# intel/QATzip

Measured on AMD Instinct MI355X. Metric: compress + decompress GB/s (input bytes), QZ_DEFLATE_GZIP_EXT L1, 64 KB chunks, higher is better.
Workload: dtype u8

## Files before the change

### qatzip_amd/csrc/qzk_common.h

```cpp
#ifndef QZK_COMMON_H
#define QZK_COMMON_H
#include <stdint.h>

#ifdef QZ_SIM
#include "hipsim.h"
#define QZ_DEV static inline
#define QZ_KERNEL static void
#define QZ_KERNEL_MAX(n) static void
#define QZ_KERNEL_OCC(n, w) static void
#define QZ_LDS static
#define QZ_CONST static const
#else
#include <hip/hip_runtime.h>
#define QZ_DEV static __device__ __forceinline__
#define QZ_KERNEL static __global__ void
#define QZ_KERNEL_MAX(n) static __global__ void __launch_bounds__(n)
#define QZ_KERNEL_OCC(n, w) static __global__ void __launch_bounds__(n, w)
#define QZ_LDS __shared__
#define QZ_CONST static __device__ const

QZ_DEV uint64_t qz_ballot(bool p) { return __ballot(p); }
QZ_DEV uint32_t qz_shfl(uint32_t v, int src) { return (uint32_t)__shfl((int)v, src, 64); }
QZ_DEV uint32_t qz_readlane(uint32_t v, int src) { return (uint32_t)__builtin_amdgcn_readlane((int)v, src); }
QZ_DEV uint32_t qz_readfirstlane(uint32_t v) { return (uint32_t)__builtin_amdgcn_readfirstlane((int)v); }
QZ_DEV uint32_t qz_writelane(uint32_t old, uint32_t val, int sel) { return (int)(threadIdx.x & 63) == sel ? val : old; }
QZ_DEV void qz_wave_sync()
{
    __builtin_amdgcn_fence(__ATOMIC_RELEASE, "workgroup");
    __builtin_amdgcn_wave_barrier();
    __builtin_amdgcn_fence(__ATOMIC_ACQUIRE, "workgroup");
}
QZ_DEV void qz_lds_sync()
{
    __builtin_amdgcn_fence(__ATOMIC_ACQ_REL, "wavefront");
    __builtin_amdgcn_wave_barrier();
}
QZ_DEV void qz_block_sync() { __syncthreads(); }
QZ_DEV int qz_lane() { return (int)(threadIdx.x & 63); }
QZ_DEV uint8_t qz_ld8_l2(const uint8_t *p) { return __hip_atomic_load(p, __ATOMIC_RELAXED, __HIP_MEMORY_SCOPE_AGENT); }
#endif
#ifdef QZ_SIM
static inline void qz_lds_sync() { qz_wave_sync(); }
static inline uint32_t qz_writelane(uint32_t old, uint32_t val, int sel) { return qz_lane() == sel ? val : old; }
static inline uint8_t qz_ld8_l2(const uint8_t *p) { return *p; }
#endif

#ifndef QZ_SIM
QZ_DEV uint32_t qz_wave_incl_scan(uint32_t v)
{
    v += (uint32_t)__builtin_amdgcn_update_dpp(0, (int)v, 0x111, 0xf, 0xf, false);
    v += (uint32_t)__builtin_amdgcn_update_dpp(0, (int)v, 0x112, 0xf, 0xf, false);
    v += (uint32_t)__builtin_amdgcn_update_dpp(0, (int)v, 0x114, 0xf, 0xf, false);
    v += (uint32_t)__builtin_amdgcn_update_dpp(0, (int)v, 0x118, 0xf, 0xf, false);
    v += (uint32_t)__builtin_amdgcn_update_dpp(0, (int)v, 0x142, 0xa, 0xf, false);
    v += (uint32_t)__builtin_amdgcn_update_dpp(0, (int)v, 0x143, 0xc, 0xf, false);
    return v;
}
#else
static inline uint32_t qz_wave_incl_scan(uint32_t v)
{
    const int lane = qz_lane();
    for (int d = 1; d < 64; d <<= 1) {
        uint32_t o = qz_shfl(v, lane - d);
        if (lane >= d) v += o;
    }
    return v;
}
#endif

QZ_DEV int qz_popc64(uint64_t v) { return __builtin_popcountll(v); }
QZ_DEV int qz_ctz64(uint64_t v) { return __builtin_ctzll(v); }
QZ_DEV int qz_ctz32(uint32_t v) { return __builtin_ctz(v); }
QZ_DEV int qz_msb64(uint64_t v) { return 63 - __builtin_clzll(v); }
QZ_DEV uint64_t qz_below(int l) { return l >= 64 ? ~0ull : ((1ull << l) - 1); }

typedef struct __attribute__((packed, aligned(1))) { uint32_t v; } qz_u32u;
typedef struct __attribute__((packed, aligned(1))) { uint16_t v; } qz_u16u;
QZ_DEV uint32_t qz_ld32(const uint8_t *p) { return ((const qz_u32u *)p)->v; }
QZ_DEV uint32_t qz_ld16(const uint8_t *p) { return ((const qz_u16u *)p)->v; }

QZ_DEV uint32_t qz_uniform(uint32_t v) { return qz_readfirstlane(v); }

#endif
```

### qatzip_amd/csrc/qzk_deflate_lz77.h

```cpp
#ifndef QZK_DEFLATE_LZ77_H
#define QZK_DEFLATE_LZ77_H
#include "qzk_common.h"
#include "qzk_crcmath.h"

#define QZK_WSIZE 32768
#define QZK_MAXDIST 32506
#define QZK_MINLOOK 262
#define QZK_LITBUF 32767
#define QZK_MAXBLK 20
#define QZK_CAP 16
#define QZK_WLIM 61
#define QZK_NICE 8
#define QZK_MAXINS 4
#define QZK_HSIZE 65536
#ifndef QZK_CNBLOG
#define QZK_CNBLOG (-1)
#endif
#if QZK_CNBLOG >= 0
#define QZK_CNB (1 << QZK_CNBLOG)
#else
#define QZK_CNB 0
#endif
#ifndef QZK_PF
#define QZK_PF (QZK_CNB ? 1 : 0)
#endif
#ifndef QZK_PF_MINL
#define QZK_PF_MINL 30
#endif
#ifndef QZK_NSLOT
#define QZK_NSLOT 256
#endif
#ifndef QZK_RING
#define QZK_RING 4096
#endif
#ifndef QZK_K1_OCC
#define QZK_K1_OCC 5
#endif
#define QZK_RINGW (QZK_RING / 4)
#ifndef QZK_NSLOT2
#define QZK_NSLOT2 128
#endif
#ifndef QZK_NSLOT3
#if QZK_CNB
#define QZK_NSLOT3 0
#else
#define QZK_NSLOT3 128
#endif
#endif
#define QZK_K1_PARSEW (2 * QZK_NSLOT + QZK_RINGW + 4 + QZK_NSLOT2 + QZK_NSLOT3 + 3 * QZK_CNB)
#ifndef QZK_K1_WAVES
#define QZK_K1_WAVES 4
#endif

#ifndef QZK_K1_TABGRP
#define QZK_K1_TABGRP 5
#endif
#define QZK_K1_TABW (QZK_K1_WAVES * QZK_K1_TABGRP)
#define QZK_K1_TABROWS(wgs) ((((wgs) + 8u * QZK_K1_TABGRP - 1) / (8u * QZK_K1_TABGRP)) * 8u)

typedef struct __attribute__((aligned(16))) { uint32_t w0, w1, w2, ep; } qzk_bkt;
typedef uint32_t qzk_u32x4 __attribute__((vector_size(16)));

QZ_DEV qzk_u32x4 qzk_ld_bkt(const qzk_bkt *p)
{
#ifdef QZ_SIM
    return *(const qzk_u32x4 *)p;
#else
    qzk_u32x4 v;
    asm volatile("global_load_dwordx4 %0, %1, off sc1\n\ts_waitcnt vmcnt(0)" : "=v"(v) : "v"(p) : "memory");
    return v;
#endif
}

QZ_DEV void qzk_ld_bkt_ahead(qzk_u32x4 *v, const qzk_bkt *p)
{
#ifdef QZ_SIM
    *v = *(const qzk_u32x4 *)p;
#else
    asm volatile("global_load_dwordx4 %0, %1, off sc1" : "+v"(*v) : "v"(p) : "memory");
#endif
}
QZ_DEV void qzk_wait_ahead(qzk_u32x4 *v)
{
#ifdef QZ_SIM
    (void)v;
#else
    asm volatile("s_waitcnt vmcnt(0)" : "+v"(*v) : : "memory");
#endif
}

#ifdef QZ_SIM
static unsigned long qzk_sim_count[2];
#define QZK_SIMC(k) do { if (qz_lane() == 0) qzk_sim_count[k]++; } while (0)
#else
#define QZK_SIMC(k) do { } while (0)
#endif
#if defined(QZK_PROF) && !defined(QZ_SIM)
#define QZK_T(k) do { uint64_t t_ = __builtin_readcyclecounter(); prof[k] += t_ - tprev; tprev = t_; } while (0)
#define QZK_C(k, v) do { prof[k] += (uint64_t)(v); } while (0)
#else
#define QZK_T(k) do { } while (0)
#define QZK_C(k, v) do { } while (0)
#endif

typedef struct {
    uint32_t nsym;
    uint32_t nfull;
    uint32_t bstart[QZK_MAXBLK];
    uint32_t can_store;
    uint32_t n;
#ifdef QZK_PROF
    uint64_t prof[24];
#endif
} qzk_lzmeta;

#define QZK_CDESC_FINAL 0x80000000u
QZ_DEV uint32_t qzk_chunk_len(const uint32_t *cdesc, uint32_t chunk, uint64_t src_len, uint32_t chunk_sz)
{
    if (cdesc) return cdesc[chunk] & ~QZK_CDESC_FINAL;
    const uint64_t coff = (uint64_t)chunk * chunk_sz;
    return (uint32_t)((src_len - coff) < chunk_sz ? (src_len - coff) : chunk_sz);
}

QZ_DEV uint32_t qzk_ld32g(const uint8_t *src, uint64_t off, uint64_t src_len)
{
    if (off + 4 <= src_len) return qz_ld32(src + off);
    uint32_t v = 0;
    for (int k = 0; k < 4; k++) if (off + k < src_len) v |= (uint32_t)src[off + k] << (8 * k);
    return v;
}

QZ_DEV uint32_t qzk_ld32g_fast(const uint8_t *src, uint64_t off, uint64_t src_len)
{
    return off + 4 <= src_len ? qz_ld32(src + off) : qzk_ld32g(src, off, src_len);
}

QZ_DEV uint32_t qzk_alignbyte(uint32_t hi, uint32_t lo, uint32_t s)
{
#ifdef QZ_SIM
    return (uint32_t)((((uint64_t)hi << 32) | lo) >> (8 * s));
#else
    return __builtin_amdgcn_alignbyte(hi, lo, s);
#endif
}

QZ_DEV int qzk_wave_matchlen(const uint8_t *src, uint64_t src_len, uint64_t a, uint64_t b, int maxlen, int lane)
{
    for (int off = 0; off < maxlen; off += 256) {
        int o = off + 4 * lane;
        bool act = o < maxlen;
        uint32_t x = 0;
        if (act) x = qzk_ld32g(src, a + o, src_len) ^ qzk_ld32g(src, b + o, src_len);
        uint64_t mm = qz_ballot(act && x != 0);
        if (mm) {
            int f = qz_ctz64(mm);
            uint32_t xf = qz_readlane(x, f);
            int len = off + 4 * f + (qz_ctz32(xf) >> 3);
            return len < maxlen ? len : maxlen;
        }
    }
    return maxlen;
}

QZ_DEV void qzk_lz77_chunk(const uint8_t *src, uint64_t src_len, uint32_t chunk_sz, uint32_t chunk,
                           uint8_t *sym_lc, uint16_t *sym_dist, qzk_lzmeta *meta, qzk_bkt *tab, uint32_t epoch,
                           const uint32_t *cdesc, uint32_t *lds, const qzk_k1crc_lds *crcT, uint32_t *crc_slot)
{
    uint32_t *const slot = lds, *const scnt = lds + QZK_NSLOT, *const ring = lds + 2 * QZK_NSLOT, *const slot2 = ring + QZK_RINGW + 4;
    uint32_t *const slot3 = slot2 + QZK_NSLOT2; (void)slot3;
#if QZK_CNB
    uint32_t *const ctag = slot3 + QZK_NSLOT3, *const cpos = ctag + QZK_CNB;
#pragma nounroll
    for (uint32_t i = (uint32_t)qz_lane(); i < QZK_CNB; i += 64) ctag[i] = 0;
#endif
    uint32_t rhi = 0;
    uint32_t crc_acc = 0;
    uint32_t rnext = qzk_ld32g_fast(src, (uint64_t)chunk * chunk_sz + 4 * (uint32_t)qz_lane(), src_len);
#define QZK_RING16(dst, ca) do { const uint32_t r_ = (ca) & (QZK_RING - 1), i_ = r_ >> 2, s_ = r_ & 3; \
        const uint32_t d0_ = ring[i_], d1_ = ring[i_ + 1], d2_ = ring[i_ + 2], d3_ = ring[i_ + 3], d4_ = ring[i_ + 4]; \
        (dst)[0] = qzk_alignbyte(d1_, d0_, s_); (dst)[1] = qzk_alignbyte(d2_, d1_, s_); \
        (dst)[2] = qzk_alignbyte(d3_, d2_, s_); (dst)[3] = qzk_alignbyte(d4_, d3_, s_); } while (0)
#define QZK_RING4(ca) ({ const uint32_t r_ = (ca) & (QZK_RING - 1), i_ = r_ >> 2; \
        qzk_alignbyte(ring[i_ + 1], ring[i_], r_ & 3); })
#define QZK_AHEAD (64 + 258 + 6)

    const int lane = qz_lane();
    const uint64_t coff = (uint64_t)chunk * chunk_sz;
    const uint32_t n = qzk_chunk_len(cdesc, chunk, src_len, chunk_sz);
    uint8_t *olc = sym_lc;
    uint16_t *odist = sym_dist;
    qzk_lzmeta *mt = meta + chunk;
    auto wave_matchlen = [&](uint32_t ca, uint32_t cb, int maxlen) -> int {
        const bool near = (int64_t)cb >= (int64_t)rhi - QZK_RING;
        for (int off = 0; off < maxlen; off += 256) {
            const int o = off + 4 * lane;
            const bool act = o < maxlen;
            uint32_t x = 0;
            if (act) x = QZK_RING4(ca + (uint32_t)o) ^ (near ? QZK_RING4(cb + (uint32_t)o) : qzk_ld32g(src, coff + cb + (uint32_t)o, src_len));
            const uint64_t mm = qz_ballot(act && x != 0);
            if (mm) {
                const int f = qz_ctz64(mm);
                const uint32_t xf = qz_readlane(x, f);
                const int len = off + 4 * f + (qz_ctz32(xf) >> 3);
                return len < maxlen ? len : maxlen;
            }
        }
        return maxlen;
    };

    qz_lds_sync();

    uint32_t base = 0;
    uint32_t fill = n < 65536u ? n : 65536u;
    uint32_t avail_in = n - fill;
    uint32_t pos = 0;
    uint32_t nsym = 0, nfull = 0, cur_bstart = 0, can_store = 0;
    mt->bstart[0] = 0;
#if QZK_PF
    qzk_u32x4 pf = {0, 0, 0, 0};
    uint64_t pf_okm = 0;
    uint32_t pf_base = 0, pf_mark = 0, wcount = 0;
    bool pf_lost = false;
    uint64_t dPm = 0, dSTm = 0;
    uint32_t dnsym = 0, dv_sym = 0, dv_h = 0, dv_e0 = 0, dv_e1 = 0, dv_e2 = 0;
#define QZK_DEFERRED_STORES() do { \
        if ((dPm >> lane) & 1) { const uint32_t i_ = dnsym + (uint32_t)qz_popc64(dPm & qz_below(lane)); \
                                 olc[i_] = (uint8_t)dv_sym; odist[i_] = (uint16_t)(dv_sym >> 8); } \
        if ((dSTm >> lane) & 1) { const qzk_u32x4 e_ = {dv_e0, dv_e1, dv_e2, epoch}; *(qzk_u32x4 *)&tab[(size_t)dv_h * QZK_K1_TABW] = e_; } \
        dPm = 0; dSTm = 0; } while (0)
    bool pf_live = false;
#endif
#if defined(QZK_PROF) && !defined(QZ_SIM)
    uint64_t prof[24] = {0}; uint64_t tprev = __builtin_readcyclecounter();
#endif

    for (;;) {
        uint32_t look = fill - pos;
        if (look < QZK_MINLOOK) {
            if (pos - base >= (uint32_t)(QZK_WSIZE + QZK_MAXDIST)) {
                base += QZK_WSIZE;
#if QZK_CNB
                qz_lds_sync();
#pragma nounroll
                for (uint32_t i = (uint32_t)lane; i < 2 * QZK_CNB; i += 64) {
                    const uint32_t v = cpos[i];
                    const int a = (int)(v & 0xffffu) - QZK_WSIZE, b = (int)(v >> 16) - QZK_WSIZE;
                    cpos[i] = (uint32_t)(a > 0 ? a : 0) | (uint32_t)(b > 0 ? b : 0) << 16;
                }
                qz_lds_sync();
#endif
            }
            if (avail_in) {
                uint32_t more = 65536u - (fill - base);
                uint32_t rd = avail_in < more ? avail_in : more;
                fill += rd; avail_in -= rd;
            }
            look = fill - pos;
            if (look == 0) break;
        }

        QZK_T(0); QZK_C(8, 1);
#if QZK_PF
        qzk_wait_ahead(&pf);
        QZK_T(17);
        QZK_DEFERRED_STORES();
        QZK_T(18);
#endif
        const uint32_t B = pos - base;
        const uint32_t p = B + (uint32_t)lane;
        const uint32_t pa = pos + (uint32_t)lane;
        const int avail = pa < fill ? (int)(fill - pa) : 0;
        const bool canh = avail >= 3;
        const bool guard = coff + pos + 64 + 2 * QZK_CAP > src_len;
        uint32_t w0 = 0, w1 = 0, w2 = 0, w3 = 0;
        {
            if (rhi < pos + QZK_AHEAD) {
                do {
                    const uint32_t a = rhi + 4 * (uint32_t)lane;
                    const uint32_t ri = (a >> 2) & (QZK_RINGW - 1);
                    ring[ri] = rnext;
                    if (ri < 4) ring[ri + QZK_RINGW] = rnext;
                    if (crcT && a + 4 <= n) crc_acc = qzk_k1crc_step(crcT, crc_acc, rnext);
                    rhi += 256;
                    rnext = qzk_ld32g_fast(src, coff + a + 256, src_len);
                } while (rhi < pos + QZK_AHEAD);
                qz_lds_sync();
            }
            uint32_t w[4];
            QZK_RING16(w, pa);
            w0 = w[0]; w1 = w[1]; w2 = w[2]; w3 = w[3];
        }
        const uint32_t h = (((w0 & 0xf) << 12) ^ (((w0 >> 8) & 0xff) << 6) ^ ((w0 >> 16) & 0xff)) & 0xffff;
        const uint32_t bucket = h;
        const uint32_t key = h & (QZK_NSLOT - 1);

        int nvalid = look < 64 ? (int)look : 64;
        int lim = nvalid < QZK_WLIM ? nvalid : QZK_WLIM;
        {
            int lstop;
            int first_short = (int)look - (QZK_MINLOOK - 1);
            if (first_short < 0) first_short = 0;
            if (avail_in) lstop = first_short;
            else {
                int sl = (int)(QZK_WSIZE + QZK_MAXDIST) - (int)B;
                lstop = first_short > sl ? first_short : sl;
            }
            if (lstop < 1) lstop = 1;
            if (lim > lstop) lim = lstop;
        }
        QZK_T(1);
        qz_lds_sync();
        qzk_u32x4 ev = {0, 0, 0, 0};
#if QZK_CNB
        const uint32_t cset = ((h * 40503u) >> (16 - QZK_CNBLOG)) & (QZK_CNB - 1);
        const uint32_t ct = ctag[cset], cp0 = cpos[cset], cp1 = cpos[QZK_CNB + cset];
        const bool chit = canh && ct == (h | 0x10000u);
        QZK_C(8, (uint64_t)qz_popc64(qz_ballot(chit)) << 32);
#if QZK_PF
        bool evhave = false;
        int limdata = 64;
        {
            const uint32_t sh = pos - pf_base;
            if (pf_live && !pf_lost && sh < 64u - (QZK_PF_MINL + 3)) {
                const int sl = lane + (int)sh;
                const uint32_t a0 = qz_shfl(pf[0], sl), a1 = qz_shfl(pf[1], sl), a2 = qz_shfl(pf[2], sl), a3 = qz_shfl(pf[3], sl);
                if (canh && !chit && sl < 64 && ((pf_okm >> (sl & 63)) & 1) && slot[key] != (pf_mark | h) && scnt[(h >> 8) & (QZK_NSLOT - 1)] != (pf_mark | h)) {
                    ev[0] = a0; ev[1] = a1; ev[2] = a2; ev[3] = a3; evhave = true;
                }
            }
            const bool lack = canh && !chit && !evhave;
            const uint64_t LACK = qz_ballot(lack);
            if (LACK) {
                const int fl = qz_ctz64(LACK);
                if (fl < QZK_PF_MINL + 3) { if (lack) { ev = qzk_ld_bkt(&tab[(size_t)bucket * QZK_K1_TABW]); evhave = true; } QZK_C(15, 1ull << 32); QZK_SIMC(0); }
                else limdata = fl - 3;
            }
        }
#else
        const bool evhave = canh && !chit;
        if (canh && !chit) ev = qzk_ld_bkt(&tab[(size_t)bucket * QZK_K1_TABW]);
#endif
#if QZK_PF
        if (lim > limdata) lim = limdata;
        QZK_SIMC(1);
#endif
        QZK_T(16);
        const bool ev_ok = ev[3] == epoch;
        uint32_t q0 = ev_ok ? ev[0] & 0xffffffu : 0, q1 = ev_ok ? (ev[0] >> 24) | ((ev[1] & 0xffffu) << 8) : 0,
                 q2 = ev_ok ? (ev[1] >> 16) | ((ev[2] & 0xffu) << 16) : 0, q3 = ev_ok ? ev[2] >> 8 : 0;
        if (chit) {
            q0 = (cp0 & 0xffffu) ? base + (cp0 & 0xffffu) : 0; q1 = (cp0 >> 16) ? base + (cp0 >> 16) : 0;
            q2 = (cp1 & 0xffffu) ? base + (cp1 & 0xffffu) : 0; q3 = (cp1 >> 16) ? base + (cp1 >> 16) : 0;
        }
#else
        if (canh) ev = qzk_ld_bkt(&tab[(size_t)bucket * QZK_K1_TABW]);
        const bool ev_ok = ev[3] == epoch;
        const uint32_t q0 = ev_ok ? ev[0] & 0xffffffu : 0, q1 = ev_ok ? (ev[0] >> 24) | ((ev[1] & 0xffffu) << 8) : 0,
                       q2 = ev_ok ? (ev[1] >> 16) | ((ev[2] & 0xffu) << 16) : 0, q3 = ev_ok ? ev[2] >> 8 : 0;
#endif
        const uint32_t lo = base + (p > QZK_MAXDIST ? p - QZK_MAXDIST : 0);
        const int maxlen = avail < 258 ? avail : 258;
        const int nice = avail < QZK_NICE ? avail : QZK_NICE;
        int best_len = 2; uint32_t best_c = 0;
        int l0 = 0, l1 = 0, l2 = 0, l3 = 0;
        bool suspect;
        int nc; uint32_t c0, c1, c2, c3;
        {
            uint32_t x[4][4];
            const bool ok0 = canh && q0 > base && pa - q0 <= QZK_MAXDIST;
            const bool ok1 = ok0 && q1 > lo;
            const bool ok2 = ok1 && q2 > lo;
            const bool ok3 = ok2 && q3 > lo;
            c0 = ok0 ? q0 : pa; c1 = ok1 ? q1 : pa; c2 = ok2 ? q2 : pa; c3 = ok3 ? q3 : pa;
            QZK_RING16(x[0], c0); QZK_RING16(x[1], c1); QZK_RING16(x[2], c2); QZK_RING16(x[3], c3);
#define QZK_LDF(k, ck) do { const uint32_t ca_ = (ck); if ((int64_t)ca_ < (int64_t)rhi - QZK_RING) { const uint64_t g_ = coff + ca_; \
        if (!guard) { x[k][0] = qz_ld32(src + g_); x[k][1] = qz_ld32(src + g_ + 4); x[k][2] = qz_ld32(src + g_ + 8); x[k][3] = qz_ld32(src + g_ + 12); } \
        else { x[k][0] = qzk_ld32g(src, g_, src_len); x[k][1] = qzk_ld32g(src, g_ + 4, src_len); x[k][2] = qzk_ld32g(src, g_ + 8, src_len); x[k][3] = qzk_ld32g(src, g_ + 12, src_len); } } } while (0)
#ifndef QZK_EXP_NOFAR
            QZK_LDF(0, c0); QZK_LDF(1, c1); QZK_LDF(2, c2); QZK_LDF(3, c3);
#endif
#undef QZK_LDF
            nc = (int)ok0 + (int)ok1 + (int)ok2 + (int)ok3;
            QZK_T(2);
            const uint32_t key2 = (h >> (16 - 8)) & (QZK_NSLOT2 - 1);
#if QZK_NSLOT3
            const uint32_t key3 = ((h * 40503u) >> 12) & (QZK_NSLOT3 - 1);
            if (canh) slot3[key3] = 0xffffffffu;
#endif
            if (canh) { slot[key] = 0xffffffffu; scnt[key] = 0; slot2[key2] = 0xffffffffu; }
            qz_lds_sync();
            if (canh) { atomicMin(&slot[key], ((uint32_t)lane << 16) | h); atomicAdd(&scnt[key], 1u); atomicMin(&slot2[key2], (uint32_t)lane); }
#if QZK_NSLOT3
            if (canh) atomicMin(&slot3[key3], (uint32_t)lane);
#endif
            qz_lds_sync();
            {
                const uint32_t sv = canh ? slot[key] : 0, sc = canh ? scnt[key] : 0, s2 = canh ? slot2[key2] : 0;
                suspect = canh && (sv >> 16) != (uint32_t)lane && !(sc == 2 && (sv & 0xffff) != h) && s2 != (uint32_t)lane;
#if QZK_NSLOT3
                if (suspect && slot3[key3] == (uint32_t)lane) suspect = false;
#endif
            }
            bool done = false;
            for (int k = 0; k < 4; k++) {
                const uint32_t ck = k == 0 ? c0 : k == 1 ? c1 : k == 2 ? c2 : c3;
                int len = 0;
                if (k < nc) {
                    uint32_t d;
                    len = QZK_CAP;
                    d = w3 ^ x[k][3]; if (d) len = 12 + (qz_ctz32(d) >> 3);
                    d = w2 ^ x[k][2]; if (d) len = 8 + (qz_ctz32(d) >> 3);
                    d = w1 ^ x[k][1]; if (d) len = 4 + (qz_ctz32(d) >> 3);
                    d = w0 ^ x[k][0]; if (d) len = (qz_ctz32(d) >> 3);
                    if (len > maxlen) len = maxlen;
                    if (!done) {
                        if (len > best_len) { best_len = len; best_c = ck; }
                        if (len >= nice) done = true;
                    }
                }
                if (k == 0) l0 = len; else if (k == 1) l1 = len; else if (k == 2) l2 = len; else l3 = len;
            }
        }
        uint32_t mlen = best_len >= 3 ? (uint32_t)best_len : 0;
        uint32_t mdist = mlen ? pa - best_c : 0;
        const bool capped = (best_len == QZK_CAP) && (maxlen > QZK_CAP);
        const bool exact0 = nc > 0 && pa - c0 == QZK_MAXDIST;

        QZK_T(3);
        const uint64_t CANH = qz_ballot(canh);
        const uint64_t CAPM = qz_ballot(capped);
        const uint64_t CX = qz_ballot(suspect) | CAPM;
        const uint64_t NOLIT = qz_ballot(mlen != 0) | CX;

        QZK_T(4);
#if QZK_PF
        {
            pf_base = pos + (uint32_t)lim; pf_live = true;
            pf_mark = 0x80000000u | wcount << 16; wcount = (wcount + 1) & 0x7fffu;
            const uint32_t ppa = pf_base + (uint32_t)lane;
            const bool pcanh = ppa + 3 <= fill;
            const uint32_t pw = QZK_RING4(ppa);
            const uint32_t ph = (((pw & 0xf) << 12) ^ (((pw >> 8) & 0xff) << 6) ^ ((pw >> 16) & 0xff)) & 0xffff;
            const uint32_t ps = ((ph * 40503u) >> (16 - QZK_CNBLOG)) & (QZK_CNB - 1);
            const uint32_t pct = ctag[ps], pc0 = cpos[ps], pc1 = cpos[QZK_CNB + ps];
            const uint32_t g0 = (pc0 & 0xffffu) ? base + (pc0 & 0xffffu) : 0, g1 = (pc0 >> 16) ? base + (pc0 >> 16) : 0,
                           g2 = (pc1 & 0xffffu) ? base + (pc1 & 0xffffu) : 0, g3 = (pc1 >> 16) ? base + (pc1 >> 16) : 0;
            pf[0] = g0 | (g1 << 24); pf[1] = (g1 >> 8) | (g2 << 16); pf[2] = (g2 >> 16) | (g3 << 8); pf[3] = epoch;
            if (pcanh && pct != (ph | 0x10000u)) qzk_ld_bkt_ahead(&pf, &tab[(size_t)ph * QZK_K1_TABW]);
            pf_okm = qz_ballot(pcanh);
        }
#endif
        uint64_t Pm = 0;
        uint64_t SHm = qz_ballot(mlen >= 3 && mlen <= QZK_MAXINS && avail - (int)mlen >= 3), S4m = qz_ballot(mlen == 4);
        int l = 0;
        while (l < lim) {
            uint64_t cxr = CX >> l;
            int nextc = cxr ? l + qz_ctz64(cxr) : 64;
            int stop = nextc < lim ? nextc : lim;
            while (l < stop) {
                const uint64_t nl = (NOLIT | (1ull << 63)) >> l;
                int e = l + qz_ctz64(nl);
                if (e > stop) e = stop;
                const uint32_t ml = qz_readlane(mlen, e);
                const int isM = e < stop ? 1 : 0;
                Pm |= ((1ull << (e - l + isM)) - 1) << l;
                l = e + (isM ? (int)ml : 0);
            }
            if (l >= lim || l != nextc) continue;
            QZK_T(5); QZK_C(9, 1);
            {
                const uint32_t h_l = qz_readlane(h, l);
                const uint64_t earlier = qz_ballot(canh && h == h_l) & qz_below(l);
                const uint32_t ml_l = qz_readlane(mlen, l);
                if (earlier == 0 && !((CAPM >> l) & 1)) {
                    QZK_C(15, 1);
                    Pm |= 1ull << l;
                    l += ml_l ? (int)ml_l : 1;
                    QZK_T(6);
                    continue;
                }
                const int avail_l = (int)look - l;
                const int maxlen_l = avail_l < 258 ? avail_l : 258;
                const int nice_l = avail_l < QZK_NICE ? avail_l : QZK_NICE;
                int cnt = 0, bl = 2; uint32_t bd = 0; bool fin = false;
                bool had_intra = false;
                if (earlier) {
                    const uint64_t ps = Pm & SHm;
                    const uint64_t I = (Pm & CANH) | (ps << 1) | (ps << 2) | ((ps & S4m) << 3);
                    uint64_t Sh = earlier & I;
                    if (B == 0) Sh &= ~1ull;
                    had_intra = Sh != 0;
                    if (Sh) {
                        const uint32_t a0 = qz_readlane(w0, l), a1 = qz_readlane(w1, l), a2 = qz_readlane(w2, l), a3 = qz_readlane(w3, l);
                        while (Sh && cnt < 4 && !fin) {
                            int j = qz_msb64(Sh);
                            Sh &= ~(1ull << j);
                            int len = QZK_CAP;
                            {
                                uint32_t d;
                                d = a3 ^ qz_readlane(w3, j); if (d) len = 12 + (qz_ctz32(d) >> 3);
                                d = a2 ^ qz_readlane(w2, j); if (d) len = 8 + (qz_ctz32(d) >> 3);
                                d = a1 ^ qz_readlane(w1, j); if (d) len = 4 + (qz_ctz32(d) >> 3);
                                d = a0 ^ qz_readlane(w0, j); if (d) len = (qz_ctz32(d) >> 3);
                            }
                            if (len > maxlen_l) len = maxlen_l;
                            if (len == QZK_CAP && maxlen_l > QZK_CAP)
                                len = wave_matchlen(pos + (uint32_t)l, pos + (uint32_t)j, maxlen_l);
                            cnt++;
                            if (len > bl) { bl = len; bd = (uint32_t)(l - j); }
                            if (len >= nice_l) fin = true;
                        }
                    }
                }
                const int nc_l = (int)qz_readlane((uint32_t)nc, l);
                const bool ex_l = qz_readlane((uint32_t)exact0, l) != 0;
                if (!fin && !(had_intra && ex_l)) {
                    for (int k = 0; k < nc_l && cnt < 4 && !fin; k++) {
                        const uint32_t ck = qz_readlane(k == 0 ? c0 : k == 1 ? c1 : k == 2 ? c2 : c3, l);
                        int len = (int)qz_readlane((uint32_t)(k == 0 ? l0 : k == 1 ? l1 : k == 2 ? l2 : l3), l);
                        if (len == QZK_CAP && maxlen_l > QZK_CAP)
                            len = wave_matchlen(pos + (uint32_t)l, ck, maxlen_l);
                        cnt++;
                        if (len > bl) { bl = len; bd = (pos + (uint32_t)l) - ck; }
                        if (len >= nice_l) fin = true;
                    }
                }
                uint32_t nl = bl >= 3 ? (uint32_t)bl : 0;
                if (lane == l) { mlen = nl; mdist = nl ? bd : 0; }
                {
                    const uint64_t bit = 1ull << l;
                    SHm = (nl >= 3 && nl <= QZK_MAXINS && avail_l - (int)nl >= 3) ? SHm | bit : SHm & ~bit;
                    S4m = nl == 4 ? S4m | bit : S4m & ~bit;
                }
                Pm |= 1ull << l;
                l += nl ? (int)nl : 1;
            }
            QZK_T(6);
        }

        QZK_T(5);
        const uint64_t ps = Pm & SHm;
        const uint64_t I = (Pm & CANH) | (ps << 1) | (ps << 2) | ((ps & S4m) << 3);
        const bool isP = (Pm >> lane) & 1, isI = (I >> lane) & 1;

        const uint32_t rank = (uint32_t)qz_popc64(Pm & qz_below(lane));
        const uint32_t idx = nsym + rank;
        const uint32_t step = mlen ? mlen : 1;
        if (isP) {
#if QZK_PF
            dv_sym = (mlen ? mlen - 3 : (w0 & 0xff)) | mdist << 8;
#else
            olc[idx] = (uint8_t)(mlen ? mlen - 3 : (w0 & 0xff));
            odist[idx] = (uint16_t)mdist;
#endif
        }
        {
            const bool closes = isP && ((idx + 1) % QZK_LITBUF == 0);
            const uint64_t cm = qz_ballot(closes);
            if (cm) {
                int f = qz_ctz64(cm);
                uint32_t nb = qz_readlane(pa + step, f);
                if (cur_bstart >= base) can_store |= 1u << nfull;
                nfull++;
                cur_bstart = nb;
                if (nfull < QZK_MAXBLK) mt->bstart[nfull] = nb;
            }
        }
#if QZK_PF
        dPm = Pm; dnsym = nsym;
#endif
        nsym += (uint32_t)qz_popc64(Pm);

        QZK_T(7);
        uint32_t n0 = pa, n1 = q0, n2 = q1, n3 = q2;
        bool store = isI;
        {
            uint64_t todo = I & qz_ballot(suspect);
            QZK_C(10, qz_popc64(todo)); QZK_C(11, qz_popc64(Pm));
            while (todo) {
                const int j = qz_msb64(todo);
                uint32_t b_j = qz_readlane(bucket, j);
                const uint64_t same = qz_ballot(canh && bucket == b_j) & I;
                todo &= ~same;
                uint64_t mates = same & qz_below(j);
                uint32_t m1 = 0, m2 = 0, m3 = 0;
                int nf = 1;
                while (mates && nf < 4) {
                    const int m = qz_msb64(mates);
                    mates &= ~(1ull << m);
                    const uint32_t mp = pos + (uint32_t)m;
                    if (nf == 1) m1 = mp; else if (nf == 2) m2 = mp; else m3 = mp;
                    nf++;
                }
                if (lane == j) {
                    if (nf == 2) { n1 = m1; n2 = q0; n3 = q1; }
                    else if (nf == 3) { n1 = m1; n2 = m2; n3 = q0; }
                    else if (nf == 4) { n1 = m1; n2 = m2; n3 = m3; }
                }
                if (((same >> lane) & 1) && lane < j) store = false;
            }
        }
#if QZK_PF
        dSTm = qz_ballot(store); dv_h = bucket;
        dv_e0 = n0 | (n1 << 24); dv_e1 = (n1 >> 8) | (n2 << 16); dv_e2 = (n2 >> 16) | (n3 << 8);
#else
        if (store) {
            const qzk_u32x4 e = {n0 | (n1 << 24), (n1 >> 8) | (n2 << 16), (n2 >> 16) | (n3 << 8), epoch};
            *(qzk_u32x4 *)&tab[(size_t)bucket * QZK_K1_TABW] = e;
        }
#endif
#if QZK_CNB
        {
            const bool ralloc = evhave && !isI;
            const uint32_t mark = (store ? 0x20040u : 0x20000u) | (uint32_t)lane;
#if QZK_PF
            {
                const uint32_t mk = pf_mark | h, key3 = (h >> 8) & (QZK_NSLOT - 1);
                if (store) slot[key] = mk;
                qz_lds_sync();
                const bool second = store && slot[key] != mk;
                if (second) scnt[key3] = mk;
                qz_lds_sync();
                pf_lost = qz_ballot(second && scnt[key3] != mk) != 0;
            }
#endif
            if (ralloc) ctag[cset] = mark;
            qz_lds_sync();
            if (store) ctag[cset] = mark;
            qz_lds_sync();
            if ((store || ralloc) && ctag[cset] == mark) {
                const uint32_t e0 = store ? n0 : q0, e1 = store ? n1 : q1, e2 = store ? n2 : q2, e3 = store ? n3 : q3;
                const uint32_t r0 = e0 > base ? e0 - base : 0, r1 = e1 > base ? e1 - base : 0, r2 = e2 > base ? e2 - base : 0,
                               r3 = e3 > base ? e3 - base : 0;
                cpos[cset] = r0 | r1 << 16; cpos[QZK_CNB + cset] = r2 | r3 << 16;
                ctag[cset] = h | 0x10000u;
            }
        }
#endif
        pos += (uint32_t)l;
        QZK_T(12);
    }

#if QZK_PF
    qzk_wait_ahead(&pf);
    QZK_DEFERRED_STORES();
#undef QZK_DEFERRED_STORES
#endif
    if (crcT) {
        for (; rhi < n; rhi += 256) {
            const uint32_t a = rhi + 4 * (uint32_t)lane;
            if (a + 4 <= n) crc_acc = qzk_k1crc_step(crcT, crc_acc, rnext);
            rnext = qzk_ld32g_fast(src, coff + a + 256, src_len);
        }
        const uint32_t n4 = n & ~3u;
        const uint32_t mine = n4 > 4u * (uint32_t)lane ? (n4 - 4u * (uint32_t)lane + 252u) >> 8 : 0;
        uint32_t part = 0;
        if (mine) part = qzk_multmodp(qzk_x2nmodp(crcT->x2n, n4 - (4u * (uint32_t)lane + 4u + 256u * (mine - 1)), 3), crc_acc);
        for (int d = 32; d >= 1; d >>= 1) part ^= qz_shfl(part, lane ^ d);
        if (n & 3u) {
            uint32_t c = 0xffffffffu;
            for (uint32_t i = n4; i < n; i++) c = qzk_crc_byte(c, src[coff + i]);
            part = qzk_multmodp(qzk_x2nmodp(crcT->x2n, n & 3u, 3), part) ^ ~c;
        }
        *crc_slot = part;
    }
    if (cur_bstart >= base) can_store |= 1u << nfull;
    mt->nsym = nsym; mt->nfull = nfull; mt->can_store = can_store; mt->n = n;
#if defined(QZK_PROF) && !defined(QZ_SIM)
    for (int k = 0; k < 24; k++) mt->prof[k] = prof[k];
#endif
#undef QZK_RING16
#undef QZK_RING4
}

#endif
```

Measured before the change: 66.27.

## Split LZ77 window loop into unguarded and guarded phases, branchless candidate matching

The per-window body becomes a lambda templated on a compile-time guard flag. Windows far enough from the chunk end run without bounds-checked loads, and only the tail runs the guarded variant. Addressing is rebased to a 32-bit chunk-relative pointer. Several per-lane predicates are turned into wave ballots computed once (CANH, SUSP, EX0, STm), LDS slot updates run unconditionally, and far-candidate loads are skipped wave-wide when no lane needs them. The aim is to cut branch divergence, 64-bit address math and redundant ballots in the hot loop, at the cost of code size and register pressure from duplicating the body.

New measurement: 65.61. About the same (-1.0%).

```diff
diff --git a/qatzip_amd/csrc/qzk_common.h b/qatzip_amd/csrc/qzk_common.h
--- a/qatzip_amd/csrc/qzk_common.h
+++ b/qatzip_amd/csrc/qzk_common.h
@@ -21,6 +21,7 @@
 
 QZ_DEV uint64_t qz_ballot(bool p) { return __ballot(p); }
 QZ_DEV uint32_t qz_shfl(uint32_t v, int src) { return (uint32_t)__shfl((int)v, src, 64); }
+QZ_DEV uint32_t qz_shfl64(uint32_t v, int src) { return (uint32_t)__builtin_amdgcn_ds_bpermute(src << 2, (int)v); }
 QZ_DEV uint32_t qz_readlane(uint32_t v, int src) { return (uint32_t)__builtin_amdgcn_readlane((int)v, src); }
 QZ_DEV uint32_t qz_readfirstlane(uint32_t v) { return (uint32_t)__builtin_amdgcn_readfirstlane((int)v); }
 QZ_DEV uint32_t qz_writelane(uint32_t old, uint32_t val, int sel) { return (int)(threadIdx.x & 63) == sel ? val : old; }
@@ -41,6 +42,7 @@
 #endif
 #ifdef QZ_SIM
 static inline void qz_lds_sync() { qz_wave_sync(); }
+static inline uint32_t qz_shfl64(uint32_t v, int src) { return qz_shfl(v, src); }
 static inline uint32_t qz_writelane(uint32_t old, uint32_t val, int sel) { return qz_lane() == sel ? val : old; }
 static inline uint8_t qz_ld8_l2(const uint8_t *p) { return *p; }
 #endif
diff --git a/qatzip_amd/csrc/qzk_deflate_lz77.h b/qatzip_amd/csrc/qzk_deflate_lz77.h
--- a/qatzip_amd/csrc/qzk_deflate_lz77.h
+++ b/qatzip_amd/csrc/qzk_deflate_lz77.h
@@ -135,6 +135,18 @@
     return off + 4 <= src_len ? qz_ld32(src + off) : qzk_ld32g(src, off, src_len);
 }
 
+QZ_DEV uint32_t qzk_ld32c(const uint8_t *csrc, uint32_t off, uint32_t end)
+{
+    if (off + 4 <= end) return qz_ld32(csrc + off);
+    uint32_t v = 0;
+    for (uint32_t k = 0; k < 4; k++) if (off + k < end) v |= (uint32_t)csrc[off + k] << (8 * k);
+    return v;
+}
+QZ_DEV uint32_t qzk_ld32c_fast(const uint8_t *csrc, uint32_t off, uint32_t end)
+{
+    return off + 4 <= end ? qz_ld32(csrc + off) : qzk_ld32c(csrc, off, end);
+}
+
 QZ_DEV uint32_t qzk_alignbyte(uint32_t hi, uint32_t lo, uint32_t s)
 {
 #ifdef QZ_SIM
@@ -143,6 +155,14 @@
     return __builtin_amdgcn_alignbyte(hi, lo, s);
 #endif
 }
+
+template <bool B> struct qzk_flag { static constexpr bool value = B; };
+
+#define QZK_LEN16(w0, w1, w2, w3, x) ({ uint32_t d_ = (w3) ^ (x)[3], b_ = 12, t_; \
+        t_ = (w2) ^ (x)[2]; if (t_) { d_ = t_; b_ = 8; } \
+        t_ = (w1) ^ (x)[1]; if (t_) { d_ = t_; b_ = 4; } \
+        t_ = (w0) ^ (x)[0]; if (t_) { d_ = t_; b_ = 0; } \
+        (int)(b_ + ((d_ ? (uint32_t)qz_ctz32(d_) : 32u) >> 3)); })
 
 QZ_DEV int qzk_wave_matchlen(const uint8_t *src, uint64_t src_len, uint64_t a, uint64_t b, int maxlen, int lane)
 {
@@ -175,7 +195,14 @@
 #endif
     uint32_t rhi = 0;
     uint32_t crc_acc = 0;
-    uint32_t rnext = qzk_ld32g_fast(src, (uint64_t)chunk * chunk_sz + 4 * (uint32_t)qz_lane(), src_len);
+    const uint8_t *const csrc = src + (uint64_t)chunk * chunk_sz;
+    const uint32_t gend = src_len - (uint64_t)chunk * chunk_sz < 0x7fffffffull ? (uint32_t)(src_len - (uint64_t)chunk * chunk_sz) : 0x7fffffffu;
+    int lane = qz_lane();
+#ifndef QZ_SIM
+    asm volatile("" : "+v"(lane));
+    lane &= 63;
+#endif
+    uint32_t rnext = qzk_ld32c_fast(csrc, 4 * (uint32_t)lane, gend);
 #define QZK_RING16(dst, ca) do { const uint32_t r_ = (ca) & (QZK_RING - 1), i_ = r_ >> 2, s_ = r_ & 3; \
         const uint32_t d0_ = ring[i_], d1_ = ring[i_ + 1], d2_ = ring[i_ + 2], d3_ = ring[i_ + 3], d4_ = ring[i_ + 4]; \
         (dst)[0] = qzk_alignbyte(d1_, d0_, s_); (dst)[1] = qzk_alignbyte(d2_, d1_, s_); \
@@ -183,20 +210,21 @@
 #define QZK_RING4(ca) ({ const uint32_t r_ = (ca) & (QZK_RING - 1), i_ = r_ >> 2; \
         qzk_alignbyte(ring[i_ + 1], ring[i_], r_ & 3); })
 #define QZK_AHEAD (64 + 258 + 6)
-
-    const int lane = qz_lane();
-    const uint64_t coff = (uint64_t)chunk * chunk_sz;
+#define QZK_RLO() ((rhi > QZK_RING ? rhi : (uint32_t)QZK_RING) - QZK_RING)
+#define QZK_GUARDSPAN (QZK_AHEAD + 512)
+
     const uint32_t n = qzk_chunk_len(cdesc, chunk, src_len, chunk_sz);
     uint8_t *olc = sym_lc;
     uint16_t *odist = sym_dist;
     qzk_lzmeta *mt = meta + chunk;
-    auto wave_matchlen = [&](uint32_t ca, uint32_t cb, int maxlen) -> int {
-        const bool near = (int64_t)cb >= (int64_t)rhi - QZK_RING;
+    auto wave_matchlen = [&](auto G, uint32_t ca, uint32_t cb, int maxlen) __attribute__((always_inline)) -> int {
+        constexpr bool GUARD = decltype(G)::value;
+        const bool near = cb >= QZK_RLO();
         for (int off = 0; off < maxlen; off += 256) {
             const int o = off + 4 * lane;
             const bool act = o < maxlen;
             uint32_t x = 0;
-            if (act) x = QZK_RING4(ca + (uint32_t)o) ^ (near ? QZK_RING4(cb + (uint32_t)o) : qzk_ld32g(src, coff + cb + (uint32_t)o, src_len));
+            if (act) x = QZK_RING4(ca + (uint32_t)o) ^ (near ? QZK_RING4(cb + (uint32_t)o) : GUARD ? qzk_ld32c(csrc, cb + (uint32_t)o, gend) : qz_ld32(csrc + (cb + (uint32_t)o)));
             const uint64_t mm = qz_ballot(act && x != 0);
             if (mm) {
                 const int f = qz_ctz64(mm);
@@ -234,7 +262,7 @@
     uint64_t prof[24] = {0}; uint64_t tprev = __builtin_readcyclecounter();
 #endif
 
-    for (;;) {
+    auto loop_top = [&]() __attribute__((always_inline)) -> bool {
         uint32_t look = fill - pos;
         if (look < QZK_MINLOOK) {
             if (pos - base >= (uint32_t)(QZK_WSIZE + QZK_MAXDIST)) {
@@ -256,9 +284,14 @@
                 fill += rd; avail_in -= rd;
             }
             look = fill - pos;
-            if (look == 0) break;
-        }
-
+            if (look == 0) return false;
+        }
+        return true;
+    };
+
+    auto window = [&](auto G) __attribute__((always_inline)) -> void {
+        constexpr bool GUARD = decltype(G)::value;
+        const uint32_t look = fill - pos;
         QZK_T(0); QZK_C(8, 1);
 #if QZK_PF
         qzk_wait_ahead(&pf);
@@ -271,7 +304,7 @@
         const uint32_t pa = pos + (uint32_t)lane;
         const int avail = pa < fill ? (int)(fill - pa) : 0;
         const bool canh = avail >= 3;
-        const bool guard = coff + pos + 64 + 2 * QZK_CAP > src_len;
+        const uint64_t CANH = qz_ballot(canh);
         uint32_t w0 = 0, w1 = 0, w2 = 0, w3 = 0;
         {
             if (rhi < pos + QZK_AHEAD) {
@@ -282,7 +315,7 @@
                     if (ri < 4) ring[ri + QZK_RINGW] = rnext;
                     if (crcT && a + 4 <= n) crc_acc = qzk_k1crc_step(crcT, crc_acc, rnext);
                     rhi += 256;
-                    rnext = qzk_ld32g_fast(src, coff + a + 256, src_len);
+                    rnext = GUARD ? qzk_ld32c_fast(csrc, a + 256, gend) : qz_ld32(csrc + (a + 256));
                 } while (rhi < pos + QZK_AHEAD);
                 qz_lds_sync();
             }
@@ -363,7 +396,7 @@
         const int nice = avail < QZK_NICE ? avail : QZK_NICE;
         int best_len = 2; uint32_t best_c = 0;
         int l0 = 0, l1 = 0, l2 = 0, l3 = 0;
-        bool suspect;
+        uint64_t SUSP, EX0;
         int nc; uint32_t c0, c1, c2, c3;
         {
             uint32_t x[4][4];
@@ -373,50 +406,53 @@
             const bool ok3 = ok2 && q3 > lo;
             c0 = ok0 ? q0 : pa; c1 = ok1 ? q1 : pa; c2 = ok2 ? q2 : pa; c3 = ok3 ? q3 : pa;
             QZK_RING16(x[0], c0); QZK_RING16(x[1], c1); QZK_RING16(x[2], c2); QZK_RING16(x[3], c3);
-#define QZK_LDF(k, ck) do { const uint32_t ca_ = (ck); if ((int64_t)ca_ < (int64_t)rhi - QZK_RING) { const uint64_t g_ = coff + ca_; \
-        if (!guard) { x[k][0] = qz_ld32(src + g_); x[k][1] = qz_ld32(src + g_ + 4); x[k][2] = qz_ld32(src + g_ + 8); x[k][3] = qz_ld32(src + g_ + 12); } \
-        else { x[k][0] = qzk_ld32g(src, g_, src_len); x[k][1] = qzk_ld32g(src, g_ + 4, src_len); x[k][2] = qzk_ld32g(src, g_ + 8, src_len); x[k][3] = qzk_ld32g(src, g_ + 12, src_len); } } } while (0)
+#define QZK_LDF(k, ck, fk) do { if (fk) { \
+        if (!GUARD) { const uint8_t *g_ = csrc + (ck); x[k][0] = qz_ld32(g_); x[k][1] = qz_ld32(g_ + 4); x[k][2] = qz_ld32(g_ + 8); x[k][3] = qz_ld32(g_ + 12); } \
+        else { x[k][0] = qzk_ld32c(csrc, (ck), gend); x[k][1] = qzk_ld32c(csrc, (ck) + 4, gend); x[k][2] = qzk_ld32c(csrc, (ck) + 8, gend); x[k][3] = qzk_ld32c(csrc, (ck) + 12, gend); } } } while (0)
 #ifndef QZK_EXP_NOFAR
-            QZK_LDF(0, c0); QZK_LDF(1, c1); QZK_LDF(2, c2); QZK_LDF(3, c3);
+            {
+                const uint32_t rlo = QZK_RLO();
+                const bool f0 = c0 < rlo, f1 = c1 < rlo, f2 = c2 < rlo, f3 = c3 < rlo;
+                if (qz_ballot(f0 || f1 || f2 || f3)) { QZK_LDF(0, c0, f0); QZK_LDF(1, c1, f1); QZK_LDF(2, c2, f2); QZK_LDF(3, c3, f3); }
+            }
 #endif
 #undef QZK_LDF
             nc = (int)ok0 + (int)ok1 + (int)ok2 + (int)ok3;
+            EX0 = qz_ballot(ok0 && pa - c0 == QZK_MAXDIST);
             QZK_T(2);
             const uint32_t key2 = (h >> (16 - 8)) & (QZK_NSLOT2 - 1);
 #if QZK_NSLOT3
             const uint32_t key3 = ((h * 40503u) >> 12) & (QZK_NSLOT3 - 1);
-            if (canh) slot3[key3] = 0xffffffffu;
-#endif
-            if (canh) { slot[key] = 0xffffffffu; scnt[key] = 0; slot2[key2] = 0xffffffffu; }
+#endif
+            const uint32_t mine = canh ? ((uint32_t)lane << 16) | h : 0xffffffffu, mlane = canh ? (uint32_t)lane : 0xffffffffu;
+#if QZK_NSLOT3
+            slot3[key3] = 0xffffffffu;
+#endif
+            slot[key] = 0xffffffffu; scnt[key] = 0; slot2[key2] = 0xffffffffu;
             qz_lds_sync();
-            if (canh) { atomicMin(&slot[key], ((uint32_t)lane << 16) | h); atomicAdd(&scnt[key], 1u); atomicMin(&slot2[key2], (uint32_t)lane); }
+            atomicMin(&slot[key], mine); atomicAdd(&scnt[key], canh ? 1u : 0u); atomicMin(&slot2[key2], mlane);
 #if QZK_NSLOT3
-            if (canh) atomicMin(&slot3[key3], (uint32_t)lane);
+            atomicMin(&slot3[key3], mlane);
 #endif
             qz_lds_sync();
             {
-                const uint32_t sv = canh ? slot[key] : 0, sc = canh ? scnt[key] : 0, s2 = canh ? slot2[key2] : 0;
-                suspect = canh && (sv >> 16) != (uint32_t)lane && !(sc == 2 && (sv & 0xffff) != h) && s2 != (uint32_t)lane;
+                const uint32_t sv = slot[key], sc = scnt[key], s2 = slot2[key2];
+                bool suspect = (sv >> 16) != (uint32_t)lane && !(sc == 2 && (sv & 0xffff) != h) && s2 != (uint32_t)lane;
 #if QZK_NSLOT3
-                if (suspect && slot3[key3] == (uint32_t)lane) suspect = false;
-#endif
+                suspect = suspect && slot3[key3] != (uint32_t)lane;
+#endif
+                SUSP = qz_ballot(suspect) & CANH;
             }
             bool done = false;
             for (int k = 0; k < 4; k++) {
                 const uint32_t ck = k == 0 ? c0 : k == 1 ? c1 : k == 2 ? c2 : c3;
-                int len = 0;
-                if (k < nc) {
-                    uint32_t d;
-                    len = QZK_CAP;
-                    d = w3 ^ x[k][3]; if (d) len = 12 + (qz_ctz32(d) >> 3);
-                    d = w2 ^ x[k][2]; if (d) len = 8 + (qz_ctz32(d) >> 3);
-                    d = w1 ^ x[k][1]; if (d) len = 4 + (qz_ctz32(d) >> 3);
-                    d = w0 ^ x[k][0]; if (d) len = (qz_ctz32(d) >> 3);
-                    if (len > maxlen) len = maxlen;
-                    if (!done) {
-                        if (len > best_len) { best_len = len; best_c = ck; }
-                        if (len >= nice) done = true;
-                    }
+                const bool live = k == 0 ? ok0 : k == 1 ? ok1 : k == 2 ? ok2 : ok3;
+                int len = QZK_LEN16(w0, w1, w2, w3, x[k]);
+                if (len > maxlen) len = maxlen;
+                if (!live) len = 0;
+                if (live && !done) {
+                    if (len > best_len) { best_len = len; best_c = ck; }
+                    if (len >= nice) done = true;
                 }
                 if (k == 0) l0 = len; else if (k == 1) l1 = len; else if (k == 2) l2 = len; else l3 = len;
             }
@@ -424,12 +460,10 @@
         uint32_t mlen = best_len >= 3 ? (uint32_t)best_len : 0;
         uint32_t mdist = mlen ? pa - best_c : 0;
         const bool capped = (best_len == QZK_CAP) && (maxlen > QZK_CAP);
-        const bool exact0 = nc > 0 && pa - c0 == QZK_MAXDIST;
 
         QZK_T(3);
-        const uint64_t CANH = qz_ballot(canh);
         const uint64_t CAPM = qz_ballot(capped);
-        const uint64_t CX = qz_ballot(suspect) | CAPM;
+        const uint64_t CX = SUSP | CAPM;
         const uint64_t NOLIT = qz_ballot(mlen != 0) | CX;
 
         QZK_T(4);
@@ -470,7 +504,7 @@
             QZK_T(5); QZK_C(9, 1);
             {
                 const uint32_t h_l = qz_readlane(h, l);
-                const uint64_t earlier = qz_ballot(canh && h == h_l) & qz_below(l);
+                const uint64_t earlier = qz_ballot(h == h_l) & CANH & qz_below(l);
                 const uint32_t ml_l = qz_readlane(mlen, l);
                 if (earlier == 0 && !((CAPM >> l) & 1)) {
                     QZK_C(15, 1);
@@ -505,7 +539,7 @@
                             }
                             if (len > maxlen_l) len = maxlen_l;
                             if (len == QZK_CAP && maxlen_l > QZK_CAP)
-                                len = wave_matchlen(pos + (uint32_t)l, pos + (uint32_t)j, maxlen_l);
+                                len = wave_matchlen(G, pos + (uint32_t)l, pos + (uint32_t)j, maxlen_l);
                             cnt++;
                             if (len > bl) { bl = len; bd = (uint32_t)(l - j); }
                             if (len >= nice_l) fin = true;
@@ -513,13 +547,13 @@
                     }
                 }
                 const int nc_l = (int)qz_readlane((uint32_t)nc, l);
-                const bool ex_l = qz_readlane((uint32_t)exact0, l) != 0;
+                const bool ex_l = (EX0 >> l) & 1;
                 if (!fin && !(had_intra && ex_l)) {
                     for (int k = 0; k < nc_l && cnt < 4 && !fin; k++) {
                         const uint32_t ck = qz_readlane(k == 0 ? c0 : k == 1 ? c1 : k == 2 ? c2 : c3, l);
                         int len = (int)qz_readlane((uint32_t)(k == 0 ? l0 : k == 1 ? l1 : k == 2 ? l2 : l3), l);
                         if (len == QZK_CAP && maxlen_l > QZK_CAP)
-                            len = wave_matchlen(pos + (uint32_t)l, ck, maxlen_l);
+                            len = wave_matchlen(G, pos + (uint32_t)l, ck, maxlen_l);
                         cnt++;
                         if (len > bl) { bl = len; bd = (pos + (uint32_t)l) - ck; }
                         if (len >= nice_l) fin = true;
@@ -573,16 +607,17 @@
 
         QZK_T(7);
         uint32_t n0 = pa, n1 = q0, n2 = q1, n3 = q2;
-        bool store = isI;
+        uint64_t STm = I;
         {
-            uint64_t todo = I & qz_ballot(suspect);
+            uint64_t todo = I & SUSP;
             QZK_C(10, qz_popc64(todo)); QZK_C(11, qz_popc64(Pm));
             while (todo) {
                 const int j = qz_msb64(todo);
                 uint32_t b_j = qz_readlane(bucket, j);
-                const uint64_t same = qz_ballot(canh && bucket == b_j) & I;
+                const uint64_t same = qz_ballot(bucket == b_j) & CANH & I;
                 todo &= ~same;
                 uint64_t mates = same & qz_below(j);
+                STm &= ~mates;
                 uint32_t m1 = 0, m2 = 0, m3 = 0;
                 int nf = 1;
                 while (mates && nf < 4) {
@@ -597,11 +632,11 @@
                     else if (nf == 3) { n1 = m1; n2 = m2; n3 = q0; }
                     else if (nf == 4) { n1 = m1; n2 = m2; n3 = m3; }
                 }
-                if (((same >> lane) & 1) && lane < j) store = false;
-            }
-        }
-#if QZK_PF
-        dSTm = qz_ballot(store); dv_h = bucket;
+            }
+        }
+        const bool store = (STm >> lane) & 1;
+#if QZK_PF
+        dSTm = STm; dv_h = bucket;
         dv_e0 = n0 | (n1 << 24); dv_e1 = (n1 >> 8) | (n2 << 16); dv_e2 = (n2 >> 16) | (n3 << 8);
 #else
         if (store) {
@@ -639,7 +674,11 @@
 #endif
         pos += (uint32_t)l;
         QZK_T(12);
-    }
+    };
+
+    bool more;
+    while ((more = loop_top()) && pos + QZK_GUARDSPAN <= gend) window(qzk_flag<false>());
+    while (more) { window(qzk_flag<true>()); more = loop_top(); }
 
 #if QZK_PF
     qzk_wait_ahead(&pf);
@@ -650,16 +689,16 @@
         for (; rhi < n; rhi += 256) {
             const uint32_t a = rhi + 4 * (uint32_t)lane;
             if (a + 4 <= n) crc_acc = qzk_k1crc_step(crcT, crc_acc, rnext);
-            rnext = qzk_ld32g_fast(src, coff + a + 256, src_len);
+            rnext = qzk_ld32c_fast(csrc, a + 256, gend);
         }
         const uint32_t n4 = n & ~3u;
         const uint32_t mine = n4 > 4u * (uint32_t)lane ? (n4 - 4u * (uint32_t)lane + 252u) >> 8 : 0;
         uint32_t part = 0;
         if (mine) part = qzk_multmodp(qzk_x2nmodp(crcT->x2n, n4 - (4u * (uint32_t)lane + 4u + 256u * (mine - 1)), 3), crc_acc);
-        for (int d = 32; d >= 1; d >>= 1) part ^= qz_shfl(part, lane ^ d);
+        for (int d = 32; d >= 1; d >>= 1) part ^= qz_shfl64(part, lane ^ d);
         if (n & 3u) {
             uint32_t c = 0xffffffffu;
-            for (uint32_t i = n4; i < n; i++) c = qzk_crc_byte(c, src[coff + i]);
+            for (uint32_t i = n4; i < n; i++) c = qzk_crc_byte(c, csrc[i]);
             part = qzk_multmodp(qzk_x2nmodp(crcT->x2n, n & 3u, 3), part) ^ ~c;
         }
         *crc_slot = part;
@@ -671,6 +710,7 @@
 #endif
 #undef QZK_RING16
 #undef QZK_RING4
-}
-
-#endif
+#undef QZK_RLO
+}
+
+#endif
```
